# mirsadm/motioncam-decoder

Hardware: AMD Instinct MI355X
Metric: MPixels/s unpacked + achieved HBM GB/s %peak, 4K 12-bit, 1/2/4/8 GPUs (higher is better)
Workload: dtype u16; 1 GPU; 3840x2160 12-bit type-7 x 240 frames/GPU, Nat (smooth field + noise sigma 12); frames_per_gpu=240, width=3840, height=2160, bits=12, encoding=7, streams=1

## Files before the change

motioncam_decoder_amd/csrc/mcraw_type7.hip:

```cpp
#include <algorithm>
#include <cstdlib>

#include "mcraw_dev.h"

#include "../../include/mcraw_hip.h"

namespace mcraw {

#define TM(p, s, n, l) ((uint32_t)((p) * 8) | ((uint32_t)(s) << 8) | ((uint32_t)((1u << (n)) - 1u) << 16) | ((uint32_t)(l) << 24))
#define Z 0u
#define ROW1(k) {TM(0, k, 1, 0), Z, Z, Z}
#define ROW2(k) {TM((k) >> 2, 2 * ((k)&3), 2, 0), Z, Z, Z}
#define ROW4(k) {TM((k) >> 1, 4 * ((k)&1), 4, 0), Z, Z, Z}
#define ROW8(k) {TM(k, 0, 8, 0), Z, Z, Z}
#define ROW10(k) {TM(5 * ((k) >> 2) + ((k)&3), 0, 8, 0), Z, Z, TM(5 * ((k) >> 2) + 4, 2 * ((k)&3), 2, 0)}
__constant__ uint32_t c_tab7[9 * 8][4] = {
    {Z, Z, Z, Z}, {Z, Z, Z, Z}, {Z, Z, Z, Z}, {Z, Z, Z, Z}, {Z, Z, Z, Z}, {Z, Z, Z, Z}, {Z, Z, Z, Z}, {Z, Z, Z, Z},
    ROW1(0), ROW1(1), ROW1(2), ROW1(3), ROW1(4), ROW1(5), ROW1(6), ROW1(7),
    ROW2(0), ROW2(1), ROW2(2), ROW2(3), ROW2(4), ROW2(5), ROW2(6), ROW2(7),
    {TM(0, 0, 3, 0), Z, Z, Z}, {TM(0, 3, 3, 0), Z, Z, Z}, {TM(0, 6, 2, 0), TM(2, 6, 1, 2), Z, Z},
    {TM(1, 0, 3, 0), Z, Z, Z}, {TM(1, 3, 3, 0), Z, Z, Z}, {TM(1, 6, 2, 0), TM(2, 7, 1, 2), Z, Z},
    {TM(2, 0, 3, 0), Z, Z, Z}, {TM(2, 3, 3, 0), Z, Z, Z},
    ROW4(0), ROW4(1), ROW4(2), ROW4(3), ROW4(4), ROW4(5), ROW4(6), ROW4(7),
    {TM(0, 0, 5, 0), Z, Z, Z}, {TM(1, 0, 5, 0), Z, Z, Z}, {TM(2, 0, 5, 0), Z, Z, Z}, {TM(3, 0, 5, 0), Z, Z, Z},
    {TM(4, 0, 5, 0), Z, Z, Z}, {TM(0, 5, 3, 0), TM(3, 5, 2, 3), Z, Z}, {TM(1, 5, 3, 0), TM(4, 5, 2, 3), Z, Z},
    {TM(2, 5, 3, 0), TM(3, 7, 1, 3), TM(4, 7, 1, 4), Z},
    {TM(0, 0, 6, 0), Z, Z, Z}, {TM(1, 0, 6, 0), Z, Z, Z}, {TM(2, 0, 6, 0), Z, Z, Z}, {TM(3, 0, 6, 0), Z, Z, Z},
    {TM(4, 0, 6, 0), Z, Z, Z}, {TM(5, 0, 6, 0), Z, Z, Z},
    {TM(0, 6, 2, 0), TM(1, 6, 2, 2), TM(2, 6, 2, 4), Z}, {TM(3, 6, 2, 0), TM(4, 6, 2, 2), TM(5, 6, 2, 4), Z},
    ROW8(0), ROW8(1), ROW8(2), ROW8(3), ROW8(4), ROW8(5), ROW8(6), ROW8(7),
    ROW10(0), ROW10(1), ROW10(2), ROW10(3), ROW10(4), ROW10(5), ROW10(6), ROW10(7),
};
#undef TM
#undef Z

__device__ __forceinline__ uint32_t term_off(uint32_t t) { return t & 0xffu; }
__device__ __forceinline__ uint32_t term_shr(uint32_t t) { return (t >> 8) & 31u; }
__device__ __forceinline__ uint32_t term_mask(uint32_t t) { return __builtin_amdgcn_perm(t, t, 0x02020202u); }
__device__ __forceinline__ uint32_t term_shl(uint32_t t) { return (t >> 24) & 31u; }

struct Unpacked { uint32_t x[4]; };

template <bool ALIGNED8>
__device__ __forceinline__ uint2 lds_read8(const uint8_t *__restrict__ base, uint32_t off)
{
    if (ALIGNED8)
        return *reinterpret_cast<const uint2 *>(base + off);
    const uint32_t *w = reinterpret_cast<const uint32_t *>(base) + (off >> 2);
    const uint32_t sh = (off & 3u) * 8u;
    const uint32_t w0 = w[0], w1 = w[1], w2 = w[2];
    return make_uint2(__builtin_amdgcn_alignbit(w1, w0, sh), __builtin_amdgcn_alignbit(w2, w1, sh));
}

template <bool ALIGNED8>
__device__ __forceinline__ Unpacked unpack8(const uint8_t *__restrict__ base, uint32_t blk, uint32_t cidx, uint32_t k,
                                            const uint4 *__restrict__ s_tab)
{
    Unpacked u;
    if (cidx >= 9u) {
        const uint2 a = lds_read8<ALIGNED8>(base, blk + 16u * k);
        const uint2 b = lds_read8<ALIGNED8>(base, blk + 16u * k + 8u);
        u.x[0] = a.x; u.x[1] = a.y; u.x[2] = b.x; u.x[3] = b.y;
        return u;
    }
    const uint4 row = s_tab[cidx * 8u + k];
    uint32_t lo = 0, hi = 0;
    const uint32_t tms[3] = {row.x, row.y, row.z};
#pragma unroll
    for (int t = 0; t < 3; t++) {
        const uint32_t tm = tms[t];
        if (!ALIGNED8 && t > 0 && !__any(tm != 0u))
            continue;
        const uint2 p = lds_read8<ALIGNED8>(base, blk + term_off(tm));
        const uint32_t m = term_mask(tm);
        lo |= ((p.x >> term_shr(tm)) & m) << term_shl(tm);
        hi |= ((p.y >> term_shr(tm)) & m) << term_shl(tm);
    }
    const uint32_t th = row.w;
    uint32_t lo8 = 0, hi8 = 0;
    if (ALIGNED8 || __any(th != 0u)) {
        const uint2 ph = lds_read8<ALIGNED8>(base, blk + term_off(th));
        const uint32_t mh = term_mask(th);
        lo8 = (ph.x >> term_shr(th)) & mh;
        hi8 = (ph.y >> term_shr(th)) & mh;
    }
    u.x[0] = __builtin_amdgcn_perm(lo8, lo, 0x05010400u);
    u.x[1] = __builtin_amdgcn_perm(lo8, lo, 0x07030602u);
    u.x[2] = __builtin_amdgcn_perm(hi8, hi, 0x05010400u);
    u.x[3] = __builtin_amdgcn_perm(hi8, hi, 0x07030602u);
    return u;
}

#ifndef MCRAW_SIDE_T
#define MCRAW_SIDE_T 512
#endif
#ifndef MCRAW_SIDE_LPT
#define MCRAW_SIDE_LPT 4
#endif
#ifndef MCRAW_SIDE_LCAP
#define MCRAW_SIDE_LCAP 512
#endif
#ifndef MCRAW_SPEC_WARM
#define MCRAW_SPEC_WARM 8192
#endif
constexpr uint32_t SIDE_XL = 9;
constexpr uint32_t SIDE_OUT = 0xFFu;
constexpr uint32_t SIDE_DEAD = 0xFEu;
static_assert(ITEM_SPLIT == 2, "k7_side sums the block lengths of half a record per item");

template <int PATTERN>
__device__ __forceinline__ uint32_t swz_xor(uint32_t v)
{
    return static_cast<uint32_t>(__builtin_amdgcn_ds_swizzle(static_cast<int>(v), PATTERN));
}

__device__ __forceinline__ void lds_barrier()
{
    asm volatile("s_waitcnt lgkmcnt(0)\n\ts_barrier" ::: "memory");
}

__device__ __forceinline__ uint2 side_strides(const uint4 v, uint32_t odd)
{
    const uint32_t pick = odd ? 0x07050301u : 0x06040200u;
    uint32_t st[2];
#pragma unroll
    for (int i = 0; i < 2; i++) {
        const uint32_t h4 = i ? __builtin_amdgcn_perm(v.w, v.z, pick) : __builtin_amdgcn_perm(v.y, v.x, pick);
        const uint32_t hb = (h4 >> 4) & 0x0F0F0F0Fu;
        const uint32_t sel = hb & 0x07070707u;
        const uint32_t lo = __builtin_amdgcn_perm(0x08060504u, 0x03020100u, sel);
        const uint32_t hi = __builtin_amdgcn_perm(0x10101010u, 0x100A0A08u, sel);
        const uint32_t g = (hb >> 3) & 0x01010101u;
        const uint32_t m = byte_mask(g);
        st[i] = (((hi & m) | (lo & ~m)) << 2) + 0x01010101u;
    }
    return make_uint2(st[0], st[1]);
}

#ifdef MCRAW_DIAG
#ifndef SIDE_PROF_BLOCK
#define SIDE_PROF_BLOCK 1u
#endif
__device__ unsigned long long g_side_prof[2][256];
#define SIDE_STAMP(slot)                                                                                               \
    do {                                                                                                               \
        if (blockIdx.x == SIDE_PROF_BLOCK && (tid == 0u || tid == 64u) && tl_n_ < 255u) {                              \
            const unsigned long long now_ = __builtin_amdgcn_s_memtime();                                              \
            g_side_prof[tid ? 1 : 0][++tl_n_] = (static_cast<unsigned long long>(slot) << 48) | (now_ - stamp_);       \
            g_side_prof[tid ? 1 : 0][0] = tl_n_;                                                                        \
        }                                                                                                              \
    } while (0)
#else
#define SIDE_STAMP(slot)
#endif

template <uint32_t SIDE_T, uint32_t SIDE_LPT, uint32_t SIDE_LCAP, uint32_t SPEC_WARM, bool PARTS, bool LASTC>
__global__ __launch_bounds__(SIDE_T) __attribute__((amdgpu_waves_per_eu(4, 4))) void k7_side(const Work7 W)
{
    constexpr uint32_t SIDE_PIECE = 16 * SIDE_T * SIDE_LPT;
    constexpr uint32_t SIDE_HALF = SIDE_PIECE / 2;
    constexpr uint32_t SIDE_BYTES = SIDE_PIECE + SIDE_XL * 16 + 16;
    __shared__ __attribute__((aligned(16))) uint8_t s_b[SIDE_BYTES];
    __shared__ __attribute__((aligned(16))) uint8_t s_T[SIDE_HALF + 80];
    __shared__ __attribute__((aligned(16))) uint16_t s_L[2][SIDE_LCAP];
    __shared__ __attribute__((aligned(16))) uint16_t s_len[2][2 * SIDE_LCAP];
    __shared__ uint4 s_tab[72];
    __shared__ __attribute__((aligned(16))) uint32_t s_st[2][4];
    __shared__ uint2 s_seg[64];
    __shared__ int32_t s_err;

    const uint32_t nfr = static_cast<uint32_t>(W.n7), nsb = PARTS ? W.nsplit[0] : 1u, nsr = PARTS ? W.nsplit[1] : 1u;
    const uint32_t bq = blockIdx.x / nfr, f = blockIdx.x - bq * nfr;
    const uint32_t s = bq < nsr ? 1u : 0u, part = s ? bq : bq - nsr, nsp = s ? nsr : nsb;
    const uint32_t fs = (nsb + nsr) * f + (s ? nsb : 0u) + part;
    const uint32_t tid = threadIdx.x, lane = tid & 63u;
    const uint32_t wave = __builtin_amdgcn_readfirstlane(tid >> 6);
#ifdef MCRAW_DIAG
    const unsigned long long stamp_ = __builtin_amdgcn_s_memtime();
    uint32_t tl_n_ = 0, nsteps_ = 0;
#endif
    if (tid < 72u)
        s_tab[tid] = reinterpret_cast<const uint4 *>(c_tab7)[tid];
    if (tid < 80u)
        s_T[SIDE_HALF + tid] = static_cast<uint8_t>(SIDE_OUT);
    if (tid == 0u)
        s_err = 0;

    const Plan7 PL = W.plans[f];
    const Plan7 *P = &PL;
    int32_t *status = W.status + fs;
    const uint32_t len = P->len;
    const __amdgpu_buffer_rsrc_t rs = frame_rsrc(P->in, len);
    SIDE_STAMP(10);

    const uint4 hv = ld_b128(rs, 0);
    const uint32_t encW = __builtin_amdgcn_readfirstlane(hv.x), encH = __builtin_amdgcn_readfirstlane(hv.y);
    const uint32_t bitsOff = __builtin_amdgcn_readfirstlane(hv.z), refsOff = __builtin_amdgcn_readfirstlane(hv.w);
    const uint32_t so = s ? refsOff : bitsOff;
    const uint64_t A0 = (static_cast<uint64_t>(so) + 4u) & ~15ull;
    const uint32_t odd = (so + 4u) & 1u;
    struct Lines {
        uint4 v[SIDE_LPT], x;
    };
    auto load_piece = [&](Lines &r, uint32_t piece) {
        const uint64_t base = A0 + static_cast<uint64_t>(piece) * SIDE_PIECE;
#pragma unroll
        for (uint32_t j = 0; j < SIDE_LPT; j++) {
            const uint64_t o = base + 16ull * (tid + SIDE_T * j);
            r.v[j] = o < len ? ld_b128(rs, static_cast<uint32_t>(o)) : make_uint4(0, 0, 0, 0);
        }
        r.x = make_uint4(0, 0, 0, 0);
        if (tid < SIDE_XL) {
            const uint64_t o = base + 16ull * (SIDE_T * SIDE_LPT + tid);
            r.x = o < len ? ld_b128(rs, static_cast<uint32_t>(o)) : make_uint4(0, 0, 0, 0);
        }
    };
    Lines nx, ny;
    load_piece(nx, 0u);
    int32_t err = 0;
    uint32_t tilesX = 0, nblk = 0, R = 0;
    if (len < 16u || bitsOff > len || refsOff > len || (encW & 63u) != 0u || encW < static_cast<uint32_t>(P->width) ||
        encW == 0u || encH == 0u || (encH & 3u) != 0u ||
        static_cast<uint64_t>(encW) * encH >= (1ull << 31)) {
        err = MCRAW_E_HEADER;
    } else {
        tilesX = encW >> 6;
        nblk = 4u * tilesX * (encH >> 2);
        R = (nblk + GROUP_BLOCKS - 1u) / GROUP_BLOCKS;
        if (R > P->ngroups)
            err = E_GEOMETRY;
        else if (so + 4u > len || so + 4u < so)
            err = MCRAW_E_TRUNCATED;
        else {
            const uint32_t count = ld_u8(rs, so) | (ld_u8(rs, so + 1u) << 8) | (ld_u8(rs, so + 2u) << 16) |
                                   (ld_u8(rs, so + 3u) << 24);
            if (__builtin_amdgcn_readfirstlane(count) < nblk)
                err = MCRAW_E_SIDESTREAM;
        }
    }
    SIDE_STAMP(11);
    Frame7 *const FR = W.frames + f;
    if (s == 0u && part == 0u && tid == 0u) {
        FR->in = P->in;
        FR->out = P->out;
        FR->len = len;
        FR->width = P->width;
        FR->rows = min(static_cast<uint32_t>(P->height), encH);
        FR->tilesX = tilesX;
        FR->nblk = err ? 0u : nblk;
        FR->fast_store = P->fast_store;
        FR->encH = encH;
        FR->pstride = P->pstride;
        for (uint32_t q = err ? 0u : nsb - 1u; q < 3u; q++) {
            FR->part_item[q] = 0xFFFFFFFFu;
            FR->part_len[q] = 0u;
        }
        W.status[W.nstatus + f] = static_cast<int32_t>(encH);
    }
    if (err) {
        if (tid == 0u)
            *status = err;
        return;
    }
    constexpr uint32_t ENDX_ = 0xFFFFFFFFu;
    uint32_t m_lo = 0u, m_hi = 0xFFFFFFFFu, np_guess = 0xFFFFFFFFu;
    if (nsp > 1u) {
        const uint32_t other = s ? bitsOff : refsOff;
        const uint64_t end_guess = other > so ? other : len;
        const uint64_t npieces = (end_guess - A0 + SIDE_PIECE - 1u) / SIDE_PIECE;
        np_guess = static_cast<uint32_t>(npieces);
        m_lo = static_cast<uint32_t>(part * npieces / nsp);
        if (part + 1u < nsp)
            m_hi = static_cast<uint32_t>((part + 1u) * npieces / nsp);
    }
    uint64_t *const sync = W.sync + (static_cast<size_t>(2u * f + s) * MAX_SPLIT7 + part) * 2u;
    uint16_t *const rp_base = (PARTS && nsp > 1u && W.rpos) ? W.rpos + (static_cast<size_t>(2u * f + s) * MAX_SPLIT7 + part) * W.Rmax : nullptr;
    const __amdgpu_buffer_rsrc_t rsp = frame_rsrc(reinterpret_cast<const uint8_t *>(rp_base), rp_base ? 2u * W.Rmax : 0u);
    uint32_t rleft = 0u, rnext = 0u, rexit = ENDX_;
    bool rdead = false;
    constexpr uint32_t ENDX = ENDX_;

    uint8_t *bits = W.bits + static_cast<size_t>(f) * W.Rmax * 64u;
    uint16_t *refs = W.refs + static_cast<size_t>(f) * W.Rmax * 64u;
    uint32_t *goff = W.grp_off + static_cast<size_t>(f) * (W.Rmax * ITEM_SPLIT + 1u);

    uint32_t upc = 0;
    uint32_t bb = 0;
    uint32_t tb = 0;
    uint32_t n = 0;
    uint64_t carry = 0u;
    uint32_t n_first = 0xFFFFFFFFu;
    int32_t lane_err = 0;
    bool dead = false;
    uint32_t decode_from = 0u;
    constexpr uint32_t NOENTRY = 0xFFFFFFFEu;
    static_assert(SPEC_WARM <= SIDE_HALF, "a speculative count starts inside the piece in front of the part's first");

    auto store_bytes = [&](const Lines &r) {
#pragma unroll
        for (uint32_t j = 0; j < SIDE_LPT; j++)
            reinterpret_cast<uint4 *>(s_b)[tid + SIDE_T * j] = r.v[j];
        if (tid < SIDE_XL)
            reinterpret_cast<uint4 *>(s_b)[SIDE_T * SIDE_LPT + tid] = r.x;
// ... 299 lines not shown
                }
                if (npc > cpiece && npc == m_chi)
                    exit1 = pu - SIDE_HALF;
                if ((!spec && cnt1 >= R) || why == 3u || npc >= m_chi)
                    break;
                if (npc > cpiece) {
                    build_strides(nx, npc);
                    load_piece(nx, npc + 1u);
                    nx_piece = npc + 1u;
                    lds_barrier();
                }
                if (wave == 0u)
                    walk(lst ^ 1u, npc > cpiece ? pu - SIDE_HALF : pu, SU, spec ? SIDE_LCAP : min(R - cnt1, SIDE_LCAP), npc > cpiece);
                cpiece = npc;
                lst ^= 1u;
            }
            SIDE_STAMP(20);
            asm volatile("s_waitcnt vmcnt(0)" ::: "memory");
        }
        const auto replay_from_count = [&]() {
            if (rp_base && counted && cnt1) {
                rleft = min(cnt1, W.Rmax);
                rnext = 0u;
                rexit = exit1;
                rdead = dead1;
            }
        };
        uint32_t pn = 0u, pw = first_cand;
        const bool ok = owns0 ? true : ask(pn, pw);
        SIDE_STAMP(21);
        decode_from = m_lo;
        if (!ok) {
            if (empty) {
                decode_from = 0xFFFFFFFFu;
                if (m_hi == 0u) {
                    tell(0u, first_cand);
                    nothing_to_decode();
                    go = false;
                }
            }
        } else if (!owns0 && (pw == ENDX || pn >= R)) {
            tell(pn, ENDX);
            nothing_to_decode();
            go = false;
        } else if (empty) {
            tell(pn, pw);
            nothing_to_decode();
            go = false;
        } else if (lastp) {
            run_piece = m_lo, run_cand = owns0 ? first_cand : pw, run_n = pn;
            if (lastc && pw == entry)
                replay_from_count();
        } else if (owns0 || pw == entry) {
            const uint32_t upto = pn + cnt1;
            tell(min(upto, R), upto >= R || dead1 || exit1 == ENDX ? ENDX : exit1);
            run_piece = m_lo, run_cand = owns0 ? first_cand : entry, run_n = pn;
            replay_from_count();
        } else {
            run_piece = m_lo, run_cand = pw, run_n = pn;
        }
        if (go && run_n >= R) {
            tell(run_n, ENDX);
            nothing_to_decode();
            go = false;
        }
    }

    uint32_t cur = 0;
    uint32_t prev_n = 0, prev_total = 0;
    if (go) {
    lds_barrier();
    upc = bb = tb = run_piece;
    n = run_n;
#ifdef MCRAW_FORCE_SEGW
    segw = true;
#else
    segw = false;
#endif
    seg_valid = false;
    carry = run_piece == 0u && decode_from == 0u ? 16u : 0u;
    if (nx_piece != run_piece)
        load_piece(nx, run_piece);
    store_bytes(nx);
    SIDE_STAMP(12);
    if (!rleft)
        build_strides(nx, run_piece);
    load_piece(nx, run_piece + 1u);
    load_piece(ny, run_piece + 2u);
    uint4 rq = make_uint4(0u, 0u, 0u, 0u);
    auto rfetch = [&](uint32_t at) { rq = ld_b128_nt(rsp, 2u * (at + 8u * lane)); };
    auto replay = [&](uint32_t lst, uint32_t room) {
        const uint32_t n = min(room, rleft);
        const uint32_t w4[4] = {rq.x, rq.y, rq.z, rq.w};
        uint32_t mine = 8u, ment = 0u;
#pragma unroll
        for (int i = 7; i >= 0; i--) {
            const uint32_t idx = 8u * lane + static_cast<uint32_t>(i), e = (w4[i >> 1] >> (16 * (i & 1))) & 0xffffu;
            const bool hit = idx >= 1u && idx < n && (e & 0x8000u) != 0u;
            mine = hit ? static_cast<uint32_t>(i) : mine;
            ment = hit ? e : ment;
        }
        const unsigned long long m = __ballot(mine != 8u);
        uint32_t take = n, pu = 0u, why = 1u;
        if (m) {
            const uint32_t fl = static_cast<uint32_t>(__builtin_ctzll(m));
            take = 8u * fl + wave_lane(mine, fl);
            pu = SIDE_HALF + (wave_lane(ment, fl) & 0x7fffu);
            why = 2u;
        } else if (n == rleft) {
            if (rdead)
                why = 3u;
            else if (rexit != ENDX)
                why = 2u, pu = SIDE_HALF + rexit;
        }
        if (8u * lane < take)
            *reinterpret_cast<uint4 *>(&s_L[lst][8u * lane]) = make_uint4(rq.x & 0x7fff7fffu, rq.y & 0x7fff7fffu, rq.z & 0x7fff7fffu, rq.w & 0x7fff7fffu);
        if (lane == 0u)
            *reinterpret_cast<uint4 *>(s_st[lst]) = make_uint4(pu, take, why, 0u);
        rfetch(rnext + take);
    };
    lds_barrier();
    SIDE_STAMP(13);
    if (wave == 0u) {
        if (rleft) {
            rfetch(0u);
            replay(0u, min(R - run_n, SIDE_LCAP / 4u));
        } else
            walk(0u, run_cand, 0u, min(R - run_n, SIDE_LCAP / 4u), true);
    }
    SIDE_STAMP(14);
    while (true) {
        lds_barrier();
        SIDE_STAMP(0);
        const uint4 st4 = *reinterpret_cast<const uint4 *>(s_st[cur]);
        const uint32_t pu = __builtin_amdgcn_readfirstlane(st4.x);
        const uint32_t total = __builtin_amdgcn_readfirstlane(st4.y);
        const uint32_t why = __builtin_amdgcn_readfirstlane(st4.z);
        const uint32_t SU = __builtin_amdgcn_readfirstlane(st4.w);
        const uint32_t npc = why == 2u ? upc + 1u : upc;
        const bool last = n + total >= R || why == 3u || npc >= m_hi;
        const bool skip = upc < decode_from;
        if (!skip && n_first == 0xFFFFFFFFu)
            n_first = n;
        if (npc > upc && npc == m_hi)
            exitc = pu - SIDE_HALF;
        if (rleft) {
            rleft -= min(total, rleft);
            rnext += total;
        }
        const bool moved = upc > bb, build = !last && npc > tb && rleft == 0u;
        if (moved) {
            store_bytes(nx);
            bb = upc;
            nx = ny;
            load_piece(ny, bb + 2u);
        }
        if (build) {
            build_strides(nx, npc);
            tb = npc;
        }
        if (moved || build)
            lds_barrier();
        SIDE_STAMP(1);
        if (wave == 0u) {
            if (!last) {
                if (rleft)
                    replay(cur ^ 1u, min(R - (n + total), SIDE_LCAP));
                else
                    walk(cur ^ 1u, npc > upc ? pu - SIDE_HALF : pu, SU, min(R - (n + total), SIDE_LCAP), npc > upc);
            }
            SIDE_STAMP(2);
            if (s == 0u && prev_total)
                scan_unit(cur ^ 1u, prev_n, prev_total);
            SIDE_STAMP(5);
        } else if (!skip) {
            const uint8_t *B = s_b;
            const uint16_t *L = s_L[cur];
            constexpr uint32_t STEP = (SIDE_T / 64u - 1u) * 8u;
            uint32_t q = (wave - 1u) * 8u + sub;
            uint32_t ro_n = q < total ? 2u * L[q] + odd : 0u;
            uint32_t hd_n = *reinterpret_cast<const uint16_t *>(B + (ro_n & ~1u)) | (static_cast<uint32_t>(B[(ro_n & ~1u) + 2u]) << 16);
            for (uint32_t qb = (wave - 1u) * 8u; qb < total; qb += STEP, q += STEP) {
                const bool live = q < total;
                const uint32_t ro = ro_n;
                const uint32_t hd = hd_n >> (8u * (ro & 1u));
                ro_n = q + STEP < total ? 2u * L[q + STEP] + odd : 0u;
                hd_n = *reinterpret_cast<const uint16_t *>(B + (ro_n & ~1u)) | (static_cast<uint32_t>(B[(ro_n & ~1u) + 2u]) << 16);
                const uint32_t b0 = live ? hd & 0xffu : 0u, b1 = (hd >> 8) & 0xffu;
                const uint32_t hb = b0 >> 4, ref = ((b0 & 15u) << 8) | b1;
                Unpacked U = unpack8<false>(B, ro + 2u, cls7_of(hb), k, s_tab);
                const u16x2 rr = __builtin_bit_cast(u16x2, ref | (ref << 16));
#pragma unroll
                for (int i = 0; i < 4; i++)
                    U.x[i] = __builtin_bit_cast(uint32_t, __builtin_bit_cast(u16x2, U.x[i]) + rr);
                const uint32_t r = n + q;
                const uint32_t idx = r * 64u + 8u * k;
                if (s == 1u) {
                    if (live)
                        *reinterpret_cast<uint4 *>(refs + idx) = make_uint4(U.x[0], U.x[1], U.x[2], U.x[3]);
                    continue;
                }
                const uint32_t nvalid = live ? min(8u, nblk - min(nblk, idx)) : 0u;
                if (nvalid < 8u) {
#pragma unroll
                    for (uint32_t i = 0; i < 4u; i++)
                        U.x[i] &= nvalid >= 2u * i + 2u ? 0xffffffffu : nvalid == 2u * i + 1u ? 0xffffu : 0u;
                }
                uint32_t c[4], over = 0;
#pragma unroll
                for (uint32_t i = 0; i < 4u; i++) {
                    c[i] = __builtin_bit_cast(uint32_t, __builtin_elementwise_min(__builtin_bit_cast(u16x2, U.x[i]),
                                                                                  __builtin_bit_cast(u16x2, 0x00100010u)));
                    over |= c[i] ^ U.x[i];
                }
                if (over)
                    lane_err |= MCRAW_E_SIDESTREAM;
                const uint32_t bytes_lo = __builtin_amdgcn_perm(c[1], c[0], 0x06040200u);
                const uint32_t bytes_hi = __builtin_amdgcn_perm(c[3], c[2], 0x06040200u);
                if (live)
                    *reinterpret_cast<uint2 *>(bits + idx) = make_uint2(bytes_lo, bytes_hi);
                uint32_t l8 = 0;
#pragma unroll
                for (uint32_t i = 0; i < 2u; i++) {
                    const uint32_t v4 = i ? bytes_hi : bytes_lo;
                    const uint32_t sel = v4 & 0x07070707u;
                    const uint32_t lo = __builtin_amdgcn_perm(0x08060504u, 0x03020100u, sel);
                    const uint32_t hi = __builtin_amdgcn_perm(0x10101010u, 0x100A0A08u, sel);
                    const uint32_t g = (v4 >> 3) & 0x01010101u;
                    const uint32_t m = byte_mask(g);
                    const uint32_t l4 = ((hi & m) | (lo & ~m)) | (v4 & 0x10101010u);
                    l8 = __builtin_amdgcn_sad_u8(l4, 0u, l8);
                }
                l8 += swz_xor<0x041F>(l8);
                l8 += swz_xor<0x081F>(l8);
                if (live && (k & 3u) == 0u)
                    s_len[cur][2u * q + (k >> 2)] = static_cast<uint16_t>(l8 << 3);
            }
            SIDE_STAMP(3);
        }
        prev_n = n;
        prev_total = skip ? 0u : total;
        n += total;
        if (last) {
            dead = why == 3u && n < R && !skip;
            break;
        }
        upc = npc;
        cur ^= 1u;
    }
    tell(min(n, R), n >= R || dead || exitc == ENDX ? ENDX : exitc);
    if (s == 0u && prev_total) {
        lds_barrier();
        if (wave == 0u)
            scan_unit(cur, prev_n, prev_total);
    }
    if (tid == 0u) {
        if (dead)
            lane_err |= MCRAW_E_TRUNCATED;
        if (s == 0u) {
            const uint32_t c32 = static_cast<uint32_t>(min(carry, static_cast<uint64_t>(0xffffffffu)));
            if (n >= R && !dead && n_first != 0xFFFFFFFFu) {
                goff[ITEM_SPLIT * R] = c32;
                if (nsp == 1u && carry > len)
                    lane_err |= MCRAW_E_TRUNCATED;
            }
            if (nsp > 1u) {
                if (part + 1u < nsp)
                    FR->part_len[part] = n_first != 0xFFFFFFFFu ? c32 : 0u;
                if (part)
                    FR->part_item[part - 1u] = n_first != 0xFFFFFFFFu ? ITEM_SPLIT * n_first : 0xFFFFFFFFu;
            }
        }
    }
    }
    if (lane_err)
        atomicOr(&s_err, lane_err);
    lds_barrier();
    if (tid == 0u)
        *status = s_err;
    SIDE_STAMP(15);
#ifdef MCRAW_DIAG
    if (blockIdx.x == SIDE_PROF_BLOCK && tid == 0u)
        g_side_prof[0][255] = nsteps_;
#endif
}

constexpr int PAY_LDS = ITEM_SPAN + 16 + 32;
constexpr uint32_t PAY_CHUNKS = ITEM_SPAN / 16 + 1;

struct ItemS {
    uint32_t valid;
    uint32_t g, nblk, tilesX;
    uint32_t base16, n16, head;
    int32_t width, rows;
    uint32_t fast;
    const uint8_t *in;
    uint32_t len;
    uint16_t *out;
    size_t meta;
    uint32_t lean;
    uint32_t pstride;
};

__device__ __forceinline__ ItemS item_scalars(const Work7 &W, uint32_t item, uint32_t first_frame, uint32_t class_groups)
{
    ItemS I;
    const uint32_t per = W.Rmax * ITEM_SPLIT;
    const uint32_t cper = class_groups * ITEM_SPLIT;
    const uint32_t fc = item / cper;
    const uint32_t f = first_frame + fc;
    const uint32_t g = item - fc * cper;
    const Frame7 *F = W.frames + f;
    const uint32_t nblk = F->nblk;
    const uint32_t *grp = W.grp_off + static_cast<size_t>(f) * (per + 1u) + g;
    I.valid = g * ITEM_BLOCKS < nblk ? 1u : 0u;
    uint32_t start = 0, end = 0;
    if (I.valid) {
        start = grp[0];
        end = grp[1];
        if (W.nsplit[0] > 1u) {
            uint32_t ps = 0u, pe = 0u, sum_s = 0u;
            uint64_t e64 = end;
#pragma unroll
            for (uint32_t q = 0; q < 3u; q++) {
                const uint32_t pi = F->part_item[q];
                ps = g >= pi ? q + 1u : ps;
                pe = g + 1u >= pi && pi != 0xFFFFFFFFu ? q + 1u : pe;
            }
#pragma unroll
            for (uint32_t q = 0; q < 3u; q++) {
                const uint32_t pl = F->part_len[q];
                sum_s += q < ps ? pl : 0u;
                e64 += q < pe ? pl : 0u;
            }
            start += sum_s;
            end = static_cast<uint32_t>(e64);
            if ((g + 1u) * ITEM_BLOCKS >= nblk && e64 > F->len)
                atomicOr(W.status + (W.nsplit[0] + W.nsplit[1]) * f, MCRAW_E_TRUNCATED);
        }
    }
    I.g = g;
    I.nblk = nblk;
    I.tilesX = F->tilesX;
    I.base16 = start & ~15u;
    I.head = start - I.base16;
    I.n16 = I.valid ? min((end - min(end, I.base16) + 15u) >> 4, PAY_CHUNKS) : 0u;
    I.width = F->width;
    I.rows = static_cast<int32_t>(F->rows);
    I.fast = F->fast_store;
    I.in = F->in;
    I.len = F->len;
    I.out = F->out;
    I.meta = static_cast<size_t>(f) * W.Rmax * 64u + static_cast<size_t>(g) * ITEM_BLOCKS;
    I.lean = 0u;
    I.pstride = F->pstride;
    return I;
}

template <bool NT = false, int POST = 0>
__device__ __forceinline__ void store_px8(const ItemS &I, const Post &post, uint32_t y, uint32_t x, uint32_t p[4])
{
    const uint32_t width = static_cast<uint32_t>(I.width);
    if (y >= static_cast<uint32_t>(I.rows) || x >= width)
        return;
    if constexpr (POST >= PK_F32) {
        float_store8<NT, POST>(I.out, post, post.inv, width, I.pstride, y, x, p, min(8u, width - x), I.fast != 0u);
        return;
    } else if (POST) {
        post_store8<NT, POST>(I.out, post, width, y, x, p, min(8u, width - x), I.fast != 0u, POST != 16 && I.lean != 0u);
        return;
    }
    uint16_t *dst = I.out + static_cast<size_t>(y) * static_cast<size_t>(width) + x;
    if (I.fast && x + 8u <= width) {
        typedef uint32_t u32x4 __attribute__((ext_vector_type(4)));
        const u32x4 v = {p[0], p[1], p[2], p[3]};
        if (NT)
            store_stream16(dst, v);
        else
            *gptr<u32x4>(dst) = v;
    } else if (x + 8u <= width) {
        typedef uint32_t u32x4_u __attribute__((ext_vector_type(4), aligned(2)));
        const u32x4_u v = {p[0], p[1], p[2], p[3]};
        *gptr<u32x4_u>(dst) = v;
    } else {
        const uint32_t n = width - x;
#pragma unroll
        for (uint32_t i = 0; i < 8u; i++)
            if (i < n)
                gptr<uint16_t>(dst)[i] = static_cast<uint16_t>(p[i >> 1] >> (16u * (i & 1u)));
    }
}

template <int ABL = 0, bool NT = false, int POST = 0>
__device__ __forceinline__ void item_decode(const ItemS &I, const Post &post, uint32_t tt, uint32_t r, uint32_t k,
                                            const uint8_t *s_pay, const uint32_t *s_blk, const uint16_t *s_ref,
                                            const uint4 *s_tab)
{
    const uint32_t tile = I.g * ITEM_TILES + tt;
    if (!I.valid || tile * 4u >= I.nblk)
        return;
    const bool whole = __ballot(true) == ~0ull;
    const uint32_t ty = tile / I.tilesX, tx = tile - ty * I.tilesX;

    const uint32_t bi = 4u * tt + 2u * r;
    const uint2 mb = *reinterpret_cast<const uint2 *>(&s_blk[bi]);
    const uint32_t refs2 = *reinterpret_cast<const uint32_t *>(&s_ref[bi]);
    Unpacked A, B;
    if (ABL == 2) {
        A.x[0] = A.x[1] = A.x[2] = A.x[3] = mb.x;
        B.x[0] = B.x[1] = B.x[2] = B.x[3] = mb.y;
    } else {
        A = unpack8<true>(s_pay, mb.x & 0xffffu, mb.x >> 16, k, s_tab);
        B = unpack8<true>(s_pay, mb.y & 0xffffu, mb.y >> 16, k, s_tab);
    }

    uint32_t o[8];
    const u16x2 rr = __builtin_bit_cast(u16x2, refs2);
#pragma unroll
    for (int m = 0; m < 4; m++) {
        const uint32_t e = __builtin_amdgcn_perm(B.x[m], A.x[m], 0x05040100u);
        const uint32_t d = __builtin_amdgcn_perm(B.x[m], A.x[m], 0x07060302u);
        o[2 * m] = __builtin_bit_cast(uint32_t, __builtin_bit_cast(u16x2, e) + rr);
        o[2 * m + 1] = __builtin_bit_cast(uint32_t, __builtin_bit_cast(u16x2, d) + rr);
    }
    if (ABL == 1) {
#pragma unroll
        for (int m = 0; m < 8; m++)
            asm volatile("" ::"v"(o[m]));
        return;
    }

    const bool lo = k < 4u;
    uint32_t p0[4], p1[4];
#pragma unroll
    for (int i = 0; i < 4; i++) {
        const uint32_t send = lo ? o[4 + i] : o[i];
        const uint32_t recv = static_cast<uint32_t>(__builtin_amdgcn_ds_swizzle(static_cast<int>(send), 0x101F));
        p0[i] = lo ? o[i] : recv;
        p1[i] = lo ? recv : o[4 + i];
    }
    const uint32_t x = 64u * tx + 8u * (2u * (k & 3u) + (k >> 2));
    const uint32_t y = 4u * ty + r;
    if (POST == 14) {
        const bool in = I.fast != 0u && y + 2u < static_cast<uint32_t>(I.rows) && x + 8u <= static_cast<uint32_t>(I.width);
        if (whole && __ballot(!in) == 0ull) {
            const uint32_t lane = threadIdx.x & 63u;
            const bool has_next = k != 7u || ((tt & 3u) != 3u && tx + 1u < I.tilesX);
            const uint32_t src = k < 4u ? lane + 4u : k < 7u ? lane - 3u : has_next ? lane + 9u : lane;
            const uint32_t width = static_cast<uint32_t>(I.width);
            post_store8_merged<14>(I.out, post, width, y, x, p0, I.lean != 0u, src, has_next);
            post_store8_merged<14>(I.out, post, width, y + 2u, x, p1, I.lean != 0u, src, has_next);
            return;
        }
    }
    store_px8<NT, POST>(I, post, y, x, p0);
    store_px8<NT, POST>(I, post, y + 2u, x, p1);
}

template <int ABL, bool NT, int POST = 0>
__global__ __launch_bounds__(256) void k7_tiles(const Work7 W, uint32_t total, uint32_t first_frame, uint32_t class_groups)
{
    __shared__ __attribute__((aligned(16))) uint8_t s_pay[4][PAY_LDS];
    __shared__ uint4 s_tab[72];
    __shared__ uint32_t s_blk[4][ITEM_BLOCKS];
    __shared__ uint16_t s_ref[4][ITEM_BLOCKS];

    const uint32_t tid = threadIdx.x;
    const uint32_t lane = tid & 63u;
    const uint32_t wave = __builtin_amdgcn_readfirstlane(tid >> 6);
    const uint32_t item = (W.xcd_chunk ? xcd_chunked(blockIdx.x, gridDim.x, W.xcd_chunk) : xcd_remap(blockIdx.x, gridDim.x)) * 4u + wave;
    if (tid < 72u)
        s_tab[tid] = reinterpret_cast<const uint4 *>(c_tab7)[tid];

    ItemS I;
    I.valid = 0;
    I.n16 = 0;
    if (item < total)
        I = item_scalars(W, item, first_frame, class_groups);

    constexpr uint32_t NV = (PAY_CHUNKS + 63u) / 64u;
    const __amdgpu_buffer_rsrc_t rs = frame_rsrc(I.in, I.len);
    uint4 v[NV];
#pragma unroll
    for (uint32_t c = 0; c < NV; c++) {
        v[c] = make_uint4(0, 0, 0, 0);
        if (ABL != 3 && lane + 64u * c < I.n16)
            v[c] = ld_b128_nt(rs, I.base16 + (lane + 64u * c) * 16u);
    }
    uint32_t b = 0, r = 0;
    if (I.valid && lane < ITEM_BLOCKS && I.g * ITEM_BLOCKS + lane < I.nblk) {
        b = W.bits[I.meta + lane];
        r = W.refs[I.meta + lane];
    }
    if constexpr (POST == 12 || POST == 10 || POST == 14) {
        const uint32_t bl2 = (W.post.mode & POST_BLACK) ? ((lane & 2u) ? W.post.black23 : W.post.black01) : 0u;
        const uint32_t bl = (lane & 1u) ? bl2 >> 16 : bl2 & 0xffffu;
        const uint32_t sw = b <= 6u ? b : b <= 8u ? 8u : 10u;
        const bool real = I.valid && lane < ITEM_BLOCKS && I.g * ITEM_BLOCKS + lane < I.nblk;
        const bool fits = !real || (b <= 10u && r >= bl && r - bl + ((1u << sw) - 1u) <= (1u << POST) - 1u && r + ((1u << sw) - 1u) <= 65535u);
        I.lean = __ballot(!fits) == 0ull ? 1u : 0u;
        if (I.lean)
            r -= bl;
    }

    uint32_t tot;
    const uint32_t ex = wave_excl_scan(lane < ITEM_BLOCKS ? len7_of(b) : 0u, lane, &tot);
    if (lane < ITEM_BLOCKS) {
        s_blk[wave][lane] = (I.head + ex) | (cls7_of(b) << 16);
        s_ref[wave][lane] = static_cast<uint16_t>(r);
    }
    uint4 *pay4 = reinterpret_cast<uint4 *>(s_pay[wave]);
#pragma unroll
    for (uint32_t c = 0; c < NV; c++)
        if (lane + 64u * c < I.n16)
            pay4[lane + 64u * c] = v[c];
    __syncthreads();

#pragma unroll
    for (uint32_t q = 0; q < ITEM_TILES / 4u; q++)
        item_decode<ABL, NT, POST>(I, W.post, q * 4u + (lane >> 4), (lane >> 3) & 1u, lane & 7u, s_pay[wave], s_blk[wave],
                                   s_ref[wave], s_tab);
}


#ifdef MCRAW_DIAG
extern "C" void mcraw_diag_side_prof(unsigned long long *out, int reset)
{
    (void)hipDeviceSynchronize();
    (void)hipMemcpyFromSymbol(out, HIP_SYMBOL(g_side_prof), sizeof(g_side_prof));
    if (reset) {
        unsigned long long z[32] = {0};
        (void)hipMemcpyToSymbol(HIP_SYMBOL(g_side_prof), z, sizeof(z));
    }
}
#endif

extern "C" uint32_t mcraw_tile_order(uint32_t b, uint32_t n, uint32_t runs)
{
    return runs ? xcd_chunked(b, n, runs) : xcd_remap(b, n);
}

void launch_k7(const Work7 &W, uint32_t stage, hipStream_t st)
{
    const uint32_t n7 = static_cast<uint32_t>(W.n7);
    switch (stage) {
    case MCRAW_K7_SIDE: {
        const dim3 sgrid(n7 * (W.nsplit[0] + W.nsplit[1]));
        if (W.nsplit[0] + W.nsplit[1] > 2u && W.side_lastc)
            hipLaunchKernelGGL((k7_side<MCRAW_SIDE_T, MCRAW_SIDE_LPT, MCRAW_SIDE_LCAP, MCRAW_SPEC_WARM, true, true>), sgrid, dim3(MCRAW_SIDE_T), 0, st, W);
        else if (W.nsplit[0] + W.nsplit[1] > 2u)
            hipLaunchKernelGGL((k7_side<MCRAW_SIDE_T, MCRAW_SIDE_LPT, MCRAW_SIDE_LCAP, MCRAW_SPEC_WARM, true, false>), sgrid, dim3(MCRAW_SIDE_T), 0, st, W);
        else
            hipLaunchKernelGGL((k7_side<MCRAW_SIDE_T, MCRAW_SIDE_LPT, MCRAW_SIDE_LCAP, MCRAW_SPEC_WARM, false, false>), sgrid, dim3(MCRAW_SIDE_T), 0, st, W);
        break;
    }
    case MCRAW_K7_TILES: {
#ifdef MCRAW_DIAG
        static const int abl = []() {
            const char *e = std::getenv("MCRAW_ABLATE");
            return e ? std::atoi(e) : 0;
        }();
#endif
        for (uint32_t k = 0; k < W.nclasses; k++) {
            const uint32_t first = W.class_first[k], count = W.class_first[k + 1] - first, groups = W.class_groups[k];
            const uint32_t total = groups * ITEM_SPLIT * count;
            if (total == 0u)
                continue;
            const dim3 grid((total + 3) / 4);
            if (W.post.mode != 0u) {
                switch (post_kind(W.post.mode)) {
                case PK_F32: hipLaunchKernelGGL((k7_tiles<0, true, PK_F32>), grid, dim3(256), 0, st, W, total, first, groups); break;
                case PK_F16: hipLaunchKernelGGL((k7_tiles<0, true, PK_F16>), grid, dim3(256), 0, st, W, total, first, groups); break;
                case PK_BF16: hipLaunchKernelGGL((k7_tiles<0, true, PK_BF16>), grid, dim3(256), 0, st, W, total, first, groups); break;
                case 12: hipLaunchKernelGGL((k7_tiles<0, true, 12>), grid, dim3(256), 0, st, W, total, first, groups); break;
                case 10: hipLaunchKernelGGL((k7_tiles<0, true, 10>), grid, dim3(256), 0, st, W, total, first, groups); break;
                case 14: hipLaunchKernelGGL((k7_tiles<0, true, 14>), grid, dim3(256), 0, st, W, total, first, groups); break;
                default: hipLaunchKernelGGL((k7_tiles<0, true, 16>), grid, dim3(256), 0, st, W, total, first, groups); break;
                }
                continue;
            }
#ifdef MCRAW_DIAG
            if (abl == 1)
                hipLaunchKernelGGL((k7_tiles<1, true>), grid, dim3(256), 0, st, W, total, first, groups);
            else if (abl == 2)
                hipLaunchKernelGGL((k7_tiles<2, true>), grid, dim3(256), 0, st, W, total, first, groups);
            else if (abl == 3)
                hipLaunchKernelGGL((k7_tiles<3, true>), grid, dim3(256), 0, st, W, total, first, groups);
            else if (abl == 4)
                hipLaunchKernelGGL((k7_tiles<0, false>), grid, dim3(256), 0, st, W, total, first, groups);
            else
#endif
                hipLaunchKernelGGL((k7_tiles<0, true>), grid, dim3(256), 0, st, W, total, first, groups);
        }
        break;
    }
    }
}

}
```

Before: 1.904 million MPixels/s.

## Fetch frame header with one lane per word and issue loads before dependencies

```diff
diff --git a/motioncam_decoder_amd/csrc/mcraw_type7.hip b/motioncam_decoder_amd/csrc/mcraw_type7.hip
--- a/motioncam_decoder_amd/csrc/mcraw_type7.hip
+++ b/motioncam_decoder_amd/csrc/mcraw_type7.hip
@@ -904,58 +904,87 @@
     uint32_t pstride;
 };
 
-__device__ __forceinline__ ItemS item_scalars(const Work7 &W, uint32_t item, uint32_t first_frame, uint32_t class_groups)
-{
-    ItemS I;
+struct ItemAt {
+    uint32_t f, g;
+    const Frame7 *F;
+    const uint32_t *grp;
+    size_t meta;
+};
+
+__device__ __forceinline__ ItemAt item_at(const Work7 &W, uint32_t item, uint32_t first_frame, uint32_t class_groups)
+{
+    ItemAt A;
     const uint32_t per = W.Rmax * ITEM_SPLIT;
     const uint32_t cper = class_groups * ITEM_SPLIT;
     const uint32_t fc = item / cper;
-    const uint32_t f = first_frame + fc;
-    const uint32_t g = item - fc * cper;
-    const Frame7 *F = W.frames + f;
-    const uint32_t nblk = F->nblk;
-    const uint32_t *grp = W.grp_off + static_cast<size_t>(f) * (per + 1u) + g;
-    I.valid = g * ITEM_BLOCKS < nblk ? 1u : 0u;
+    A.f = first_frame + fc;
+    A.g = item - fc * cper;
+    A.F = W.frames + A.f;
+    A.grp = W.grp_off + static_cast<size_t>(A.f) * (per + 1u) + A.g;
+    A.meta = static_cast<size_t>(A.f) * W.Rmax * 64u + static_cast<size_t>(A.g) * ITEM_BLOCKS;
+    return A;
+}
+
+constexpr uint32_t F7_WORDS = sizeof(Frame7) / 4u;
+static_assert(sizeof(Frame7) % 4u == 0 && F7_WORDS + 2u <= 64u, "one lane per word of Frame7, two for the payload offsets");
+#define F7_WORD(member) (static_cast<uint32_t>(offsetof(Frame7, member)) / 4u)
+
+__device__ __forceinline__ uint32_t item_words(const ItemAt &A, uint32_t lane)
+{
+    const uint32_t *fw = reinterpret_cast<const uint32_t *>(A.F);
+    const uint32_t *p = lane < F7_WORDS ? fw + lane : lane < F7_WORDS + 2u ? A.grp + (lane - F7_WORDS) : fw;
+    return *gptr<const uint32_t>(p);
+}
+
+__device__ __forceinline__ ItemS item_scalars(const Work7 &W, const ItemAt &A, uint32_t hw, bool live)
+{
+    ItemS I;
+    const uint32_t f = A.f, g = A.g;
+    const uint32_t nblk = wave_lane(hw, F7_WORD(nblk));
+    const uint32_t len = wave_lane(hw, F7_WORD(len));
+    I.valid = live && g * ITEM_BLOCKS < nblk ? 1u : 0u;
     uint32_t start = 0, end = 0;
     if (I.valid) {
-        start = grp[0];
-        end = grp[1];
+        start = wave_lane(hw, F7_WORDS);
+        end = wave_lane(hw, F7_WORDS + 1u);
         if (W.nsplit[0] > 1u) {
             uint32_t ps = 0u, pe = 0u, sum_s = 0u;
             uint64_t e64 = end;
 #pragma unroll
             for (uint32_t q = 0; q < 3u; q++) {
-                const uint32_t pi = F->part_item[q];
+                const uint32_t pi = wave_lane(hw, F7_WORD(part_item) + q);
                 ps = g >= pi ? q + 1u : ps;
                 pe = g + 1u >= pi && pi != 0xFFFFFFFFu ? q + 1u : pe;
             }
 #pragma unroll
             for (uint32_t q = 0; q < 3u; q++) {
-                const uint32_t pl = F->part_len[q];
+                const uint32_t pl = wave_lane(hw, F7_WORD(part_len) + q);
                 sum_s += q < ps ? pl : 0u;
                 e64 += q < pe ? pl : 0u;
             }
             start += sum_s;
             end = static_cast<uint32_t>(e64);
-            if ((g + 1u) * ITEM_BLOCKS >= nblk && e64 > F->len)
+            if ((g + 1u) * ITEM_BLOCKS >= nblk && e64 > len)
                 atomicOr(W.status + (W.nsplit[0] + W.nsplit[1]) * f, MCRAW_E_TRUNCATED);
         }
     }
     I.g = g;
     I.nblk = nblk;
-    I.tilesX = F->tilesX;
+    I.tilesX = wave_lane(hw, F7_WORD(tilesX));
     I.base16 = start & ~15u;
     I.head = start - I.base16;
     I.n16 = I.valid ? min((end - min(end, I.base16) + 15u) >> 4, PAY_CHUNKS) : 0u;
-    I.width = F->width;
-    I.rows = static_cast<int32_t>(F->rows);
-    I.fast = F->fast_store;
-    I.in = F->in;
-    I.len = F->len;
-    I.out = F->out;
-    I.meta = static_cast<size_t>(f) * W.Rmax * 64u + static_cast<size_t>(g) * ITEM_BLOCKS;
+    I.width = static_cast<int32_t>(wave_lane(hw, F7_WORD(width)));
+    I.rows = static_cast<int32_t>(wave_lane(hw, F7_WORD(rows)));
+    I.fast = wave_lane(hw, F7_WORD(fast_store));
+    I.in = reinterpret_cast<const uint8_t *>(static_cast<uint64_t>(wave_lane(hw, F7_WORD(in))) |
+                                             static_cast<uint64_t>(wave_lane(hw, F7_WORD(in) + 1u)) << 32);
+    I.len = len;
+    I.out = reinterpret_cast<uint16_t *>(static_cast<uint64_t>(wave_lane(hw, F7_WORD(out))) |
+                                         static_cast<uint64_t>(wave_lane(hw, F7_WORD(out) + 1u)) << 32);
+    I.meta = A.meta;
     I.lean = 0u;
-    I.pstride = F->pstride;
+    I.pstride = wave_lane(hw, F7_WORD(pstride));
     return I;
 }
 
@@ -1059,6 +1088,19 @@
     store_px8<NT, POST>(I, post, y + 2u, x, p1);
 }
 
+#ifdef MCRAW_DIAG
+constexpr uint32_t TILE_PROF_N = 64, TILE_PROF_STRIDE = 3001, TILE_SLOTS = 9;
+enum { TILE_START, TILE_ARGS, TILE_FRAME, TILE_SPAN_ISSUED, TILE_META, TILE_BARRIER, TILE_SPAN_LDS, TILE_LAST_STORE, TILE_END };
+__device__ uint32_t g_tile_prof[TILE_PROF_N][4][TILE_SLOTS];
+#define TILE_STAMP(slot) tile_t_[slot] = __builtin_amdgcn_s_memtime()
+#define TILE_NEED_S(x) asm volatile("" ::"s"(x))
+#define TILE_NEED_V(x) asm volatile("" ::"v"(x))
+#else
+#define TILE_STAMP(slot)
+#define TILE_NEED_S(x)
+#define TILE_NEED_V(x)
+#endif
+
 template <int ABL, bool NT, int POST = 0>
 __global__ __launch_bounds__(256) void k7_tiles(const Work7 W, uint32_t total, uint32_t first_frame, uint32_t class_groups)
 {
@@ -1067,38 +1109,60 @@
     __shared__ uint32_t s_blk[4][ITEM_BLOCKS];
     __shared__ uint16_t s_ref[4][ITEM_BLOCKS];
 
+#ifdef MCRAW_DIAG
+    unsigned long long tile_t_[TILE_SLOTS];
+    TILE_STAMP(TILE_START);
+    TILE_NEED_S(total);
+    TILE_STAMP(TILE_ARGS);
+#endif
     const uint32_t tid = threadIdx.x;
     const uint32_t lane = tid & 63u;
     const uint32_t wave = __builtin_amdgcn_readfirstlane(tid >> 6);
-    const uint32_t item = (W.xcd_chunk ? xcd_chunked(blockIdx.x, gridDim.x, W.xcd_chunk) : xcd_remap(blockIdx.x, gridDim.x)) * 4u + wave;
-    if (tid < 72u)
-        s_tab[tid] = reinterpret_cast<const uint4 *>(c_tab7)[tid];
-
-    ItemS I;
-    I.valid = 0;
-    I.n16 = 0;
-    if (item < total)
-        I = item_scalars(W, item, first_frame, class_groups);
+    const uint32_t item0 = (W.xcd_chunk ? xcd_chunked(blockIdx.x, gridDim.x, W.xcd_chunk) : xcd_remap(blockIdx.x, gridDim.x)) * 4u + wave;
+    const bool live = item0 < total;
+    const ItemAt A = item_at(W, live ? item0 : total - 1u, first_frame, class_groups);
+
+    uint4 trow = make_uint4(0, 0, 0, 0);
+    if (wave * 64u < 72u)
+        trow = reinterpret_cast<const uint4 *>(c_tab7)[tid < 72u ? tid : 0u];
+    const uint32_t hw = item_words(A, lane);
+    uint32_t b = *gptr<const uint8_t>(W.bits + A.meta + (lane & (ITEM_BLOCKS - 1u)));
+    uint32_t r = *gptr<const uint16_t>(W.refs + A.meta + (lane & (ITEM_BLOCKS - 1u)));
+
+    ItemS I = item_scalars(W, A, hw, live);
+    TILE_NEED_S(I.base16);
+    TILE_NEED_S(I.n16);
+    TILE_NEED_S(I.len);
+    TILE_STAMP(TILE_FRAME);
 
     constexpr uint32_t NV = (PAY_CHUNKS + 63u) / 64u;
+    static_assert(PAY_CHUNKS == 64u * (NV - 1u) + 1u, "the last round of the span is one chunk (a misaligned item of raw-16 blocks only)");
     const __amdgpu_buffer_rsrc_t rs = frame_rsrc(I.in, I.len);
+    const uint32_t behind = (I.len + 3u) & ~3u;
     uint4 v[NV];
 #pragma unroll
     for (uint32_t c = 0; c < NV; c++) {
         v[c] = make_uint4(0, 0, 0, 0);
-        if (ABL != 3 && lane + 64u * c < I.n16)
-            v[c] = ld_b128_nt(rs, I.base16 + (lane + 64u * c) * 16u);
-    }
-    uint32_t b = 0, r = 0;
-    if (I.valid && lane < ITEM_BLOCKS && I.g * ITEM_BLOCKS + lane < I.nblk) {
-        b = W.bits[I.meta + lane];
-        r = W.refs[I.meta + lane];
-    }
+        const uint32_t at = lane + 64u * c < I.n16 ? I.base16 + (lane + 64u * c) * 16u : behind;
+        if (ABL == 3)
+            continue;
+        if (c + 1u < NV)
+            v[c] = ld_b128_nt(rs, at);
+        else if (I.n16 > 64u * c)
+            v[c] = ld_b128_nt(rs, at);
+    }
+    TILE_STAMP(TILE_SPAN_ISSUED);
+
+    const bool real = I.valid && lane < ITEM_BLOCKS && I.g * ITEM_BLOCKS + lane < I.nblk;
+    TILE_NEED_V(b);
+    TILE_NEED_V(r);
+    TILE_STAMP(TILE_META);
+    b = real ? b : 0u;
+    r = real ? r : 0u;
     if constexpr (POST == 12 || POST == 10 || POST == 14) {
         const uint32_t bl2 = (W.post.mode & POST_BLACK) ? ((lane & 2u) ? W.post.black23 : W.post.black01) : 0u;
         const uint32_t bl = (lane & 1u) ? bl2 >> 16 : bl2 & 0xffffu;
         const uint32_t sw = b <= 6u ? b : b <= 8u ? 8u : 10u;
-        const bool real = I.valid && lane < ITEM_BLOCKS && I.g * ITEM_BLOCKS + lane < I.nblk;
         const bool fits = !real || (b <= 10u && r >= bl && r - bl + ((1u << sw) - 1u) <= (1u << POST) - 1u && r + ((1u << sw) - 1u) <= 65535u);
         I.lean = __ballot(!fits) == 0ull ? 1u : 0u;
         if (I.lean)
@@ -1111,17 +1175,35 @@
         s_blk[wave][lane] = (I.head + ex) | (cls7_of(b) << 16);
         s_ref[wave][lane] = static_cast<uint16_t>(r);
     }
+    if (tid < 72u)
+        s_tab[tid] = trow;
+    lds_barrier();
+    TILE_STAMP(TILE_BARRIER);
+
     uint4 *pay4 = reinterpret_cast<uint4 *>(s_pay[wave]);
 #pragma unroll
     for (uint32_t c = 0; c < NV; c++)
         if (lane + 64u * c < I.n16)
             pay4[lane + 64u * c] = v[c];
-    __syncthreads();
+    __builtin_amdgcn_fence(__ATOMIC_ACQ_REL, "wavefront");
+    TILE_STAMP(TILE_SPAN_LDS);
 
 #pragma unroll
     for (uint32_t q = 0; q < ITEM_TILES / 4u; q++)
         item_decode<ABL, NT, POST>(I, W.post, q * 4u + (lane >> 4), (lane >> 3) & 1u, lane & 7u, s_pay[wave], s_blk[wave],
                                    s_ref[wave], s_tab);
+#ifdef MCRAW_DIAG
+    TILE_STAMP(TILE_LAST_STORE);
+    asm volatile("s_waitcnt vmcnt(0)" ::: "memory");
+    TILE_STAMP(TILE_END);
+    if (lane < TILE_SLOTS && blockIdx.x % TILE_PROF_STRIDE == 0u && blockIdx.x / TILE_PROF_STRIDE < TILE_PROF_N) {
+        uint32_t d = 0;
+#pragma unroll
+        for (uint32_t k = 0; k < TILE_SLOTS; k++)
+            d = lane == k ? static_cast<uint32_t>(tile_t_[k] - tile_t_[TILE_START]) : d;
+        g_tile_prof[blockIdx.x / TILE_PROF_STRIDE][wave][lane] = lane == TILE_START ? 1u : d;
+    }
+#endif
 }
 
 
@@ -1134,6 +1216,15 @@
         unsigned long long z[32] = {0};
         (void)hipMemcpyToSymbol(HIP_SYMBOL(g_side_prof), z, sizeof(z));
     }
+}
+
+extern "C" void mcraw_diag_tile_prof(uint32_t *out, uint32_t *dims)
+{
+    dims[0] = TILE_PROF_N, dims[1] = 4u, dims[2] = TILE_SLOTS;
+    if (!out)
+        return;
+    (void)hipDeviceSynchronize();
+    (void)hipMemcpyFromSymbol(out, HIP_SYMBOL(g_tile_prof), sizeof(g_tile_prof));
 }
 #endif
 
```

Result: no change. 1.888 million MPixels/s (-0.8%).

## Make tile decode waves independent: per-wave LDS handover, early exit, hoisted metadata loads

Applied to the files above, without the earlier changes.

```diff
diff --git a/motioncam_decoder_amd/csrc/mcraw_type7.hip b/motioncam_decoder_amd/csrc/mcraw_type7.hip
--- a/motioncam_decoder_amd/csrc/mcraw_type7.hip
+++ b/motioncam_decoder_amd/csrc/mcraw_type7.hip
@@ -1,4 +1,5 @@
 #include <algorithm>
+#include <cassert>
 #include <cstdlib>
 
 #include "mcraw_dev.h"
@@ -904,7 +905,9 @@
     uint32_t pstride;
 };
 
-__device__ __forceinline__ ItemS item_scalars(const Work7 &W, uint32_t item, uint32_t first_frame, uint32_t class_groups)
+static_assert(ITEM_BLOCKS * ITEM_SPLIT == 64, "bits / refs hold 64 entries per group: g * ITEM_BLOCKS + lane stays inside the frame's slice");
+__device__ __forceinline__ ItemS item_scalars(const Work7 &W, uint32_t item, uint32_t first_frame, uint32_t class_groups, uint32_t lane,
+                                              uint32_t *bits_lane, uint32_t *refs_lane)
 {
     ItemS I;
     const uint32_t per = W.Rmax * ITEM_SPLIT;
@@ -912,50 +915,50 @@
     const uint32_t fc = item / cper;
     const uint32_t f = first_frame + fc;
     const uint32_t g = item - fc * cper;
-    const Frame7 *F = W.frames + f;
-    const uint32_t nblk = F->nblk;
+    const Frame7 F = W.frames[f];
     const uint32_t *grp = W.grp_off + static_cast<size_t>(f) * (per + 1u) + g;
+    uint32_t start = grp[0], end = grp[1];
+    I.meta = static_cast<size_t>(f) * W.Rmax * 64u + static_cast<size_t>(g) * ITEM_BLOCKS;
+    if (lane < ITEM_BLOCKS) {
+        *bits_lane = W.bits[I.meta + lane];
+        *refs_lane = W.refs[I.meta + lane];
+    }
+    const uint32_t nblk = F.nblk;
     I.valid = g * ITEM_BLOCKS < nblk ? 1u : 0u;
-    uint32_t start = 0, end = 0;
-    if (I.valid) {
-        start = grp[0];
-        end = grp[1];
-        if (W.nsplit[0] > 1u) {
-            uint32_t ps = 0u, pe = 0u, sum_s = 0u;
-            uint64_t e64 = end;
-#pragma unroll
-            for (uint32_t q = 0; q < 3u; q++) {
-                const uint32_t pi = F->part_item[q];
-                ps = g >= pi ? q + 1u : ps;
-                pe = g + 1u >= pi && pi != 0xFFFFFFFFu ? q + 1u : pe;
-            }
-#pragma unroll
-            for (uint32_t q = 0; q < 3u; q++) {
-                const uint32_t pl = F->part_len[q];
-                sum_s += q < ps ? pl : 0u;
-                e64 += q < pe ? pl : 0u;
-            }
-            start += sum_s;
-            end = static_cast<uint32_t>(e64);
-            if ((g + 1u) * ITEM_BLOCKS >= nblk && e64 > F->len)
-                atomicOr(W.status + (W.nsplit[0] + W.nsplit[1]) * f, MCRAW_E_TRUNCATED);
-        }
+    if (I.valid && W.nsplit[0] > 1u) {
+        uint32_t ps = 0u, pe = 0u, sum_s = 0u;
+        uint64_t e64 = end;
+#pragma unroll
+        for (uint32_t q = 0; q < 3u; q++) {
+            const uint32_t pi = F.part_item[q];
+            ps = g >= pi ? q + 1u : ps;
+            pe = g + 1u >= pi && pi != 0xFFFFFFFFu ? q + 1u : pe;
+        }
+#pragma unroll
+        for (uint32_t q = 0; q < 3u; q++) {
+            const uint32_t pl = F.part_len[q];
+            sum_s += q < ps ? pl : 0u;
+            e64 += q < pe ? pl : 0u;
+        }
+        start += sum_s;
+        end = static_cast<uint32_t>(e64);
+        if ((g + 1u) * ITEM_BLOCKS >= nblk && e64 > F.len)
+            atomicOr(W.status + (W.nsplit[0] + W.nsplit[1]) * f, MCRAW_E_TRUNCATED);
     }
     I.g = g;
     I.nblk = nblk;
-    I.tilesX = F->tilesX;
+    I.tilesX = F.tilesX;
     I.base16 = start & ~15u;
     I.head = start - I.base16;
     I.n16 = I.valid ? min((end - min(end, I.base16) + 15u) >> 4, PAY_CHUNKS) : 0u;
-    I.width = F->width;
-    I.rows = static_cast<int32_t>(F->rows);
-    I.fast = F->fast_store;
-    I.in = F->in;
-    I.len = F->len;
-    I.out = F->out;
-    I.meta = static_cast<size_t>(f) * W.Rmax * 64u + static_cast<size_t>(g) * ITEM_BLOCKS;
+    I.width = F.width;
+    I.rows = static_cast<int32_t>(F.rows);
+    I.fast = F.fast_store;
+    I.in = F.in;
+    I.len = F.len;
+    I.out = F.out;
     I.lean = 0u;
-    I.pstride = F->pstride;
+    I.pstride = F.pstride;
     return I;
 }
 
@@ -1059,6 +1062,48 @@
     store_px8<NT, POST>(I, post, y + 2u, x, p1);
 }
 
+#ifdef MCRAW_DIAG
+constexpr uint32_t TILE_STAMP_ROWS = 2048u, TILE_STAMP_EVERY = 127u;
+__device__ unsigned long long g_tile_stamps[TILE_STAMP_ROWS][8];
+#define TILE_STAMP(slot)                                                                                               \
+    do {                                                                                                               \
+        if (stamped_)                                                                                                  \
+            ts_[slot] = __builtin_amdgcn_s_memtime();                                                                  \
+    } while (0)
+#define TILE_STAMP_WAIT(slot, what)                                                                                    \
+    do {                                                                                                               \
+        if (stamped_) {                                                                                                \
+            asm volatile("s_waitcnt " what ::: "memory");                                                              \
+            ts_[slot] = __builtin_amdgcn_s_memtime();                                                                  \
+        }                                                                                                              \
+    } while (0)
+#define TILE_STAMP_BEGIN()                                                                                             \
+    const bool stamped_ = wave == 1u && blockIdx.x % TILE_STAMP_EVERY == 0u && blockIdx.x / TILE_STAMP_EVERY < TILE_STAMP_ROWS; \
+    unsigned long long ts_[8] = {0, 0, 0, 0, 0, 0, 0, 0};                                                              \
+    TILE_STAMP(0)
+#define TILE_STAMP_END()                                                                                               \
+    do {                                                                                                               \
+        TILE_STAMP(6);                                                                                                 \
+        TILE_STAMP_WAIT(7, "vmcnt(0)");                                                                                \
+        if (stamped_ && lane == 0u)                                                                                    \
+            for (uint32_t i_ = 0; i_ < 8u; i_++)                                                                       \
+                g_tile_stamps[blockIdx.x / TILE_STAMP_EVERY][i_] = ts_[i_];                                            \
+    } while (0)
+#else
+#define TILE_STAMP(slot)
+#define TILE_STAMP_WAIT(slot, what)
+#define TILE_STAMP_BEGIN()
+#define TILE_STAMP_END()
+#endif
+
+__device__ __forceinline__ void wave_lds_handover()
+{
+    __builtin_amdgcn_fence(__ATOMIC_RELEASE, "wavefront");
+    __builtin_amdgcn_s_waitcnt(0xc07f);
+    __builtin_amdgcn_wave_barrier();
+    __builtin_amdgcn_fence(__ATOMIC_ACQUIRE, "wavefront");
+}
+
 template <int ABL, bool NT, int POST = 0>
 __global__ __launch_bounds__(256) void k7_tiles(const Work7 W, uint32_t total, uint32_t first_frame, uint32_t class_groups)
 {
@@ -1071,14 +1116,21 @@
     const uint32_t lane = tid & 63u;
     const uint32_t wave = __builtin_amdgcn_readfirstlane(tid >> 6);
     const uint32_t item = (W.xcd_chunk ? xcd_chunked(blockIdx.x, gridDim.x, W.xcd_chunk) : xcd_remap(blockIdx.x, gridDim.x)) * 4u + wave;
-    if (tid < 72u)
-        s_tab[tid] = reinterpret_cast<const uint4 *>(c_tab7)[tid];
-
-    ItemS I;
-    I.valid = 0;
-    I.n16 = 0;
-    if (item < total)
-        I = item_scalars(W, item, first_frame, class_groups);
+    if (item >= total)
+        return;
+    TILE_STAMP_BEGIN();
+
+    static_assert(sizeof(c_tab7) == 64 * 16 + 32 * 4 && sizeof(c_tab7) == sizeof(s_tab), "a 16-byte row per lane, then a dword for lanes 0-31");
+    const uint4 trow = reinterpret_cast<const uint4 *>(c_tab7)[lane];
+    uint32_t trest = 0;
+    if (lane < 32u)
+        trest = reinterpret_cast<const uint32_t *>(c_tab7)[256u + lane];
+    TILE_STAMP(1);
+    uint32_t b = 0, r = 0;
+    ItemS I = item_scalars(W, item, first_frame, class_groups, lane, &b, &r);
+    TILE_STAMP_WAIT(2, "lgkmcnt(0)");
+    if (!I.valid)
+        return;
 
     constexpr uint32_t NV = (PAY_CHUNKS + 63u) / 64u;
     const __amdgpu_buffer_rsrc_t rs = frame_rsrc(I.in, I.len);
@@ -1089,39 +1141,43 @@
         if (ABL != 3 && lane + 64u * c < I.n16)
             v[c] = ld_b128_nt(rs, I.base16 + (lane + 64u * c) * 16u);
     }
-    uint32_t b = 0, r = 0;
-    if (I.valid && lane < ITEM_BLOCKS && I.g * ITEM_BLOCKS + lane < I.nblk) {
-        b = W.bits[I.meta + lane];
-        r = W.refs[I.meta + lane];
-    }
+    TILE_STAMP(3);
+    const bool real = lane < ITEM_BLOCKS && I.g * ITEM_BLOCKS + lane < I.nblk;
+    if (!real)
+        b = r = 0u;
     if constexpr (POST == 12 || POST == 10 || POST == 14) {
         const uint32_t bl2 = (W.post.mode & POST_BLACK) ? ((lane & 2u) ? W.post.black23 : W.post.black01) : 0u;
         const uint32_t bl = (lane & 1u) ? bl2 >> 16 : bl2 & 0xffffu;
         const uint32_t sw = b <= 6u ? b : b <= 8u ? 8u : 10u;
-        const bool real = I.valid && lane < ITEM_BLOCKS && I.g * ITEM_BLOCKS + lane < I.nblk;
         const bool fits = !real || (b <= 10u && r >= bl && r - bl + ((1u << sw) - 1u) <= (1u << POST) - 1u && r + ((1u << sw) - 1u) <= 65535u);
         I.lean = __ballot(!fits) == 0ull ? 1u : 0u;
         if (I.lean)
             r -= bl;
     }
 
+    TILE_STAMP_WAIT(4, "vmcnt(0)");
     uint32_t tot;
     const uint32_t ex = wave_excl_scan(lane < ITEM_BLOCKS ? len7_of(b) : 0u, lane, &tot);
     if (lane < ITEM_BLOCKS) {
         s_blk[wave][lane] = (I.head + ex) | (cls7_of(b) << 16);
         s_ref[wave][lane] = static_cast<uint16_t>(r);
     }
+    s_tab[lane] = trow;
+    if (lane < 32u)
+        reinterpret_cast<uint32_t *>(s_tab)[256u + lane] = trest;
     uint4 *pay4 = reinterpret_cast<uint4 *>(s_pay[wave]);
 #pragma unroll
     for (uint32_t c = 0; c < NV; c++)
         if (lane + 64u * c < I.n16)
             pay4[lane + 64u * c] = v[c];
-    __syncthreads();
+    wave_lds_handover();
+    TILE_STAMP(5);
 
 #pragma unroll
     for (uint32_t q = 0; q < ITEM_TILES / 4u; q++)
         item_decode<ABL, NT, POST>(I, W.post, q * 4u + (lane >> 4), (lane >> 3) & 1u, lane & 7u, s_pay[wave], s_blk[wave],
                                    s_ref[wave], s_tab);
+    TILE_STAMP_END();
 }
 
 
@@ -1134,6 +1190,13 @@
         unsigned long long z[32] = {0};
         (void)hipMemcpyToSymbol(HIP_SYMBOL(g_side_prof), z, sizeof(z));
     }
+}
+
+extern "C" unsigned mcraw_diag_tile_stamps(unsigned long long *out)
+{
+    (void)hipDeviceSynchronize();
+    (void)hipMemcpyFromSymbol(out, HIP_SYMBOL(g_tile_stamps), sizeof(g_tile_stamps));
+    return TILE_STAMP_ROWS;
 }
 #endif
 
@@ -1168,6 +1231,7 @@
             const uint32_t total = groups * ITEM_SPLIT * count;
             if (total == 0u)
                 continue;
+            assert(groups <= W.Rmax && first + count <= n7);
             const dim3 grid((total + 3) / 4);
             if (W.post.mode != 0u) {
                 switch (post_kind(W.post.mode)) {
```

After: 1.901 million MPixels/s before, 1.855 million MPixels/s after. 0.976x the previous value.
